# fxxJuses/MICFormer

Hardware: AMD Instinct MI355X
Metric: train volumes/sec (128^3 CT+MRI pair) (higher is better)
Workload: dtype bf16; 1 GPU; MicFormer base Head(embed_dim=48, depths 2-2-6-2, heads 3-6-12-24, window 2^3, 8 classes) full train step (fwd + MDiceLoss + bwd + Adam/cosine) on 128^3 CT+MR pairs, DropPath on; local_batch=2, global_batch=2, parallelism=dp1, launch=hipGraph replay (one graph)

## Files before the change

micformer_amd/csrc/conv3_wgradx.hip:

```cpp
#include <cstdlib>
#include <mutex>

#include "common.h"
#include "gemm_dma.h"

namespace micf {

constexpr int wCS = 48;
constexpr int wDS = 20;
constexpr int wXS = 52;
constexpr int wPairs = 27 * (wCS / 16);
constexpr int wTPW = (wPairs + 3) / 4;
constexpr int wSlabFloats = 4 * wTPW * 256;

constexpr int kWgxItems = 12;
struct WgxArgs {
  const float* dy[kWgxItems];
  const float* x1[kWgxItems]; const float* x2[kWgxItems];
  int c1, c2;
  float* ws;
  float* bias_ws;
  int B, D, H, W, tiles_d, tiles_h, tiles_w, tiles_per_group, groups, slabs, xcd_order;
};

template <int TW, bool BF16>
__global__ void __launch_bounds__(256) conv3_wgradx_kernel(WgxArgs a) {
  constexpr int CH = 16 / TW, TH = 64 / TW;
  constexpr int HH = TH + 2, HW = TW + 2, HALO = 3 * HH * HW;
  extern __shared__ __attribute__((aligned(16))) float Xs[];
  const int tid = threadIdx.x, lane = tid & 63, wave = __builtin_amdgcn_readfirstlane(tid >> 6), li = lane & 15, lr = lane >> 4;
  int slab = blockIdx.x, group = blockIdx.y;
  const int item = blockIdx.z;
  if (a.xcd_order) {
    const int L = gridDim.x * gridDim.y;
    const int lin = slab + gridDim.x * group;
    const int logical = (lin % 8) * (L / 8) + lin / 8;
    slab = logical % gridDim.x;
    group = logical / gridDim.x;
  }
  const float* __restrict__ a_dy = a.dy[item];
  const float* __restrict__ a_x1 = a.x1[item];
  const float* __restrict__ a_x2 = a.x2[item];
  const int Cin = a.c1 + a.c2;
  const int cbase = slab * wCS;
  const int64_t DHW = (int64_t)a.D * a.H * a.W;

  f32x4 acc[wTPW];
#pragma unroll
  for (int p = 0; p < wTPW; ++p) acc[p] = f32x4{0.f, 0.f, 0.f, 0.f};
  float bsum = 0.f;
  int offs[wTPW];
#pragma unroll
  for (int p = 0; p < wTPW; ++p) {
    const int pair = min(wave * wTPW + p, wPairs - 1);
    const int tap = pair / (wCS / 16), ct = pair % (wCS / 16);
    const int kd = tap / 9, kh = (tap / 3) % 3, kw = tap % 3;
    offs[p] = (((kd - 1) * HH + (kh - 1)) * HW + (kw - 1)) * wXS + ct * 16;
  }

  const int ntiles = a.B * a.tiles_d * a.tiles_h * a.tiles_w;
  const int t_begin = group * a.tiles_per_group;
  const int t_end = min(ntiles, t_begin + a.tiles_per_group);
  constexpr int NQ = HALO * (wCS / 4);
  constexpr int NB = 16;
  static_assert(NQ <= 256 * NB, "one batch per tile");
  float* Dys = Xs + HALO * wXS;
  float4 v[NB], vdy;
  auto fetch = [&](int tile) {
    int q = tile;
    const int tw = q % a.tiles_w; q /= a.tiles_w;
    const int th = q % a.tiles_h; q /= a.tiles_h;
    const int d0 = q % a.tiles_d; const int b = q / a.tiles_d;
    const int h0 = th * TH, w0 = tw * TW;
#pragma unroll
    for (int u = 0; u < NB; ++u) {
      const int idx = u * 256 + tid;
      v[u] = make_float4(0.f, 0.f, 0.f, 0.f);
      if (idx < NQ) {
        const int hv = idx / (wCS / 4), g = idx % (wCS / 4);
        const int hw = hv % HW, hh = (hv / HW) % HH, hd = hv / (HW * HH);
        const int dd = d0 + hd - 1, yy = h0 + hh - 1, ww = w0 + hw - 1;
        const int c = cbase + 4 * g;
        if ((unsigned)dd < (unsigned)a.D && (unsigned)yy < (unsigned)a.H && (unsigned)ww < (unsigned)a.W && c < Cin) {
          const int64_t tok = (int64_t)b * DHW + ((int64_t)dd * a.H + yy) * a.W + ww;
          v[u] = c < a.c1 ? *reinterpret_cast<const float4*>(a_x1 + tok * a.c1 + c)
                          : *reinterpret_cast<const float4*>(a_x2 + tok * a.c2 + (c - a.c1));
        }
      }
    }
    {
      const int tk = tid >> 2, yy = h0 + tk / TW, ww = w0 + tk % TW;
      vdy = make_float4(0.f, 0.f, 0.f, 0.f);
      if (yy < a.H && ww < a.W)
        vdy = *reinterpret_cast<const float4*>(a_dy + ((int64_t)b * DHW + ((int64_t)d0 * a.H + yy) * a.W + ww) * 16 + 4 * (tid & 3));
    }
  };
  if (t_begin < t_end) fetch(t_begin);
  for (int tile = t_begin; tile < t_end; ++tile) {
    __syncthreads();
#pragma unroll
    for (int u = 0; u < NB; ++u) {
      const int idx = u * 256 + tid;
      if (idx < NQ) *reinterpret_cast<float4*>(&Xs[(idx / (wCS / 4)) * wXS + 4 * (idx % (wCS / 4))]) = v[u];
    }
    *reinterpret_cast<float4*>(&Dys[(tid >> 2) * wDS + 4 * (tid & 3)]) = vdy;
    auto load_dy = [&](int g, float (&bv)[4]) {
#pragma unroll
      for (int s = 0; s < 4; ++s) bv[s] = g < 4 ? Dys[(g * 16 + 4 * lr + s) * wDS + li] : 0.f;
    };
    __syncthreads();
    if (tile + 1 < t_end) fetch(tile + 1);
    float bv[4], bn[4];
    load_dy(0, bv);

    if constexpr (!BF16) {
#pragma unroll 1
    for (int g = 0; g < 4; ++g) {
      load_dy(g + 1, bn);
      int vox[4];
#pragma unroll
      for (int s = 0; s < 4; ++s) {
        const int j = 4 * lr + s;
        const int lh = g * CH + j / TW, lw = j % TW;
        vox[s] = ((1 * HH + lh + 1) * HW + lw + 1) * wXS + li;
      }
      if (a.bias_ws && wave == 0) bsum += bv[0] + bv[1] + bv[2] + bv[3];
#pragma unroll
      for (int s = 0; s < 4; ++s) {
#pragma unroll
        for (int p = 0; p < wTPW; ++p) {
          acc[p] = __builtin_amdgcn_mfma_f32_16x16x4f32(Xs[vox[s] + offs[p]], bv[s], acc[p], 0, 0, 0);
        }
      }
#pragma unroll
      for (int s = 0; s < 4; ++s) bv[s] = bn[s];
    }
    } else {
#pragma unroll 1
    for (int g = 0; g < 4; g += 2) {
      float b2[4];
      load_dy(g + 1, b2);
      load_dy(g + 2, bn);
      int vox[8];
#pragma unroll
      for (int s = 0; s < 8; ++s) {
        const int j = 4 * lr + (s & 3);
        const int lh = (g + (s >> 2)) * CH + j / TW, lw = j % TW;
        vox[s] = ((1 * HH + lh + 1) * HW + lw + 1) * wXS + li;
      }
      if (a.bias_ws && wave == 0) bsum += (bv[0] + bv[1] + bv[2] + bv[3]) + (b2[0] + b2[1] + b2[2] + b2[3]);
      const bf16x8 bb = to_bf16x8(make_float4(bv[0], bv[1], bv[2], bv[3]), make_float4(b2[0], b2[1], b2[2], b2[3]));
#pragma unroll
      for (int p = 0; p < wTPW; ++p) {
        const float* xp = Xs + offs[p];
        const bf16x8 ba = to_bf16x8(make_float4(xp[vox[0]], xp[vox[1]], xp[vox[2]], xp[vox[3]]),
                                    make_float4(xp[vox[4]], xp[vox[5]], xp[vox[6]], xp[vox[7]]));
        acc[p] = __builtin_amdgcn_mfma_f32_16x16x32_bf16(ba, bb, acc[p], 0, 0, 0);
      }
#pragma unroll
      for (int s = 0; s < 4; ++s) bv[s] = bn[s];
    }
    }
  }
  float* out = a.ws + (((int64_t)item * a.slabs + slab) * a.groups + group) * wSlabFloats;
#pragma unroll
  for (int p = 0; p < wTPW; ++p)
    *reinterpret_cast<float4*>(out + ((wave * wTPW + p) * 64 + lane) * 4) = make_float4(acc[p][0], acc[p][1], acc[p][2], acc[p][3]);
  if (a.bias_ws && slab == 0 && wave == 0) {
    bsum += __shfl_xor(bsum, 16, 64);
    bsum += __shfl_xor(bsum, 32, 64);
    if (lane < 16) a.bias_ws[((int64_t)item * a.groups + group) * 16 + lane] = bsum;
  }
}

constexpr int wRSB = 104;
constexpr int wDYB = 40;
typedef short s16x4x __attribute__((ext_vector_type(4)));

__device__ __forceinline__ bf16x8 tr_pair(unsigned a0, unsigned a1) {
  const s16x4x lo = __builtin_amdgcn_ds_read_tr16_b64_v4i16((__attribute__((address_space(3))) s16x4x*)(uintptr_t)a0);
  const s16x4x hi = __builtin_amdgcn_ds_read_tr16_b64_v4i16((__attribute__((address_space(3))) s16x4x*)(uintptr_t)a1);
  return bf16x8{lo[0], lo[1], lo[2], lo[3], hi[0], hi[1], hi[2], hi[3]};
}

template <int TW>
__global__ void __launch_bounds__(256) conv3_wgradx_b16_kernel(WgxArgs a) {
  constexpr int TH = 64 / TW;
  constexpr int HH = TH + 2, HW = TW + 2, HALO = 3 * HH * HW;
  extern __shared__ __attribute__((aligned(16))) char smem[];
  const int tid = threadIdx.x, lane = tid & 63, wave = __builtin_amdgcn_readfirstlane(tid >> 6), li = lane & 15, lr = lane >> 4;
  int slab = blockIdx.x, group = blockIdx.y;
  const int item = blockIdx.z;
  if (a.xcd_order) {
    const int L = gridDim.x * gridDim.y;
    const int lin = slab + gridDim.x * group;
    const int logical = (lin % 8) * (L / 8) + lin / 8;
    slab = logical % gridDim.x;
    group = logical / gridDim.x;
  }
  const float* __restrict__ a_dy = a.dy[item];
  const float* __restrict__ a_x1 = a.x1[item];
  const float* __restrict__ a_x2 = a.x2[item];
  const int Cin = a.c1 + a.c2;
  const int cbase = slab * wCS;
  const int64_t DHW = (int64_t)a.D * a.H * a.W;
  const unsigned xh = (unsigned)(uintptr_t)smem, dyl = xh + HALO * wRSB;

  f32x4 acc[wTPW];
#pragma unroll
  for (int p = 0; p < wTPW; ++p) acc[p] = f32x4{0.f, 0.f, 0.f, 0.f};
  int offs[wTPW];
#pragma unroll
  for (int p = 0; p < wTPW; ++p) {
    const int pair = min(wave * wTPW + p, wPairs - 1);
    const int tap = pair / (wCS / 16), ct = pair % (wCS / 16);
    const int kd = tap / 9, kh = (tap / 3) % 3, kw = tap % 3;
    offs[p] = (((kd - 1) * HH + (kh - 1)) * HW + (kw - 1)) * wRSB + ct * 32;
  }
  unsigned abase[2][2], bbase[2][2];
#pragma unroll
  for (int ks = 0; ks < 2; ++ks)
#pragma unroll
    for (int r = 0; r < 2; ++r) {
      const int t = 8 * lr + 4 * r + (li >> 2);
      const int lh = ks * (32 / TW) + t / TW, lw = t % TW;
      abase[ks][r] = xh + (unsigned)(((1 * HH + lh + 1) * HW + lw + 1) * wRSB + 8 * (li & 3));
      bbase[ks][r] = dyl + (unsigned)((32 * ks + t) * wDYB + 8 * (li & 3));
    }
  float4 bs = make_float4(0.f, 0.f, 0.f, 0.f);

  const int ntiles = a.B * a.tiles_d * a.tiles_h * a.tiles_w;
  const int t_begin = group * a.tiles_per_group;
  const int t_end = min(ntiles, t_begin + a.tiles_per_group);
  constexpr int NQ = HALO * (wCS / 4);
  constexpr int NB = 16;
  static_assert(NQ <= 256 * NB, "one batch per tile");
  float4 v[NB], vdy;
  auto fetch = [&](int tile) {
    int q = tile;
    const int tw = q % a.tiles_w; q /= a.tiles_w;
    const int th = q % a.tiles_h; q /= a.tiles_h;
    const int d0 = q % a.tiles_d; const int b = q / a.tiles_d;
    const int h0 = th * TH, w0 = tw * TW;
#pragma unroll
    for (int u = 0; u < NB; ++u) {
      const int idx = u * 256 + tid;
      v[u] = make_float4(0.f, 0.f, 0.f, 0.f);
      if (idx < NQ) {
        const int hv = idx / (wCS / 4), g = idx % (wCS / 4);
        const int hw = hv % HW, hh = (hv / HW) % HH, hd = hv / (HW * HH);
        const int dd = d0 + hd - 1, yy = h0 + hh - 1, ww = w0 + hw - 1;
        const int c = cbase + 4 * g;
        if ((unsigned)dd < (unsigned)a.D && (unsigned)yy < (unsigned)a.H && (unsigned)ww < (unsigned)a.W && c < Cin) {
          const int64_t tok = (int64_t)b * DHW + ((int64_t)dd * a.H + yy) * a.W + ww;
          v[u] = c < a.c1 ? *reinterpret_cast<const float4*>(a_x1 + tok * a.c1 + c)
                          : *reinterpret_cast<const float4*>(a_x2 + tok * a.c2 + (c - a.c1));
        }
      }
    }
    const int tk = tid >> 2, yy = h0 + tk / TW, ww = w0 + tk % TW;
    vdy = make_float4(0.f, 0.f, 0.f, 0.f);
    if (yy < a.H && ww < a.W)
      vdy = *reinterpret_cast<const float4*>(a_dy + ((int64_t)b * DHW + ((int64_t)d0 * a.H + yy) * a.W + ww) * 16 + 4 * (tid & 3));
  };
  typedef unsigned u32x2w __attribute__((ext_vector_type(2)));
  if (t_begin < t_end) fetch(t_begin);
  for (int tile = t_begin; tile < t_end; ++tile) {
    __syncthreads();
#pragma unroll
    for (int u = 0; u < NB; ++u) {
      const int idx = u * 256 + tid;
      if (idx < NQ)
        *reinterpret_cast<u32x2w*>(smem + (idx / (wCS / 4)) * wRSB + 8 * (idx % (wCS / 4))) = u32x2w{pack_bf16(v[u].x, v[u].y), pack_bf16(v[u].z, v[u].w)};
    }
    *reinterpret_cast<u32x2w*>(smem + HALO * wRSB + (tid >> 2) * wDYB + 8 * (tid & 3)) = u32x2w{pack_bf16(vdy.x, vdy.y), pack_bf16(vdy.z, vdy.w)};
    bs.x += vdy.x; bs.y += vdy.y; bs.z += vdy.z; bs.w += vdy.w;
    __syncthreads();
    if (tile + 1 < t_end) fetch(tile + 1);
#pragma unroll
    for (int ks = 0; ks < 2; ++ks) {
      const bf16x8 bb = tr_pair(bbase[ks][0], bbase[ks][1]);
#pragma unroll
      for (int p = 0; p < wTPW; ++p) {
        const bf16x8 ba = tr_pair(abase[ks][0] + offs[p], abase[ks][1] + offs[p]);
        acc[p] = __builtin_amdgcn_mfma_f32_16x16x32_bf16(ba, bb, acc[p], 0, 0, 0);
      }
    }
  }
  float* out = a.ws + (((int64_t)item * a.slabs + slab) * a.groups + group) * wSlabFloats;
#pragma unroll
  for (int p = 0; p < wTPW; ++p)
    *reinterpret_cast<float4*>(out + ((wave * wTPW + p) * 64 + lane) * 4) = make_float4(acc[p][0], acc[p][1], acc[p][2], acc[p][3]);
  if (a.bias_ws && slab == 0) {
#pragma unroll
    for (int d = 4; d < 64; d <<= 1) {
      bs.x += __shfl_xor(bs.x, d, 64); bs.y += __shfl_xor(bs.y, d, 64); bs.z += __shfl_xor(bs.z, d, 64); bs.w += __shfl_xor(bs.w, d, 64);
    }
    __syncthreads();
    float* red = reinterpret_cast<float*>(smem);
    if (lane < 4) *reinterpret_cast<float4*>(red + (wave * 4 + lane) * 4) = bs;
    __syncthreads();
    if (tid < 16) a.bias_ws[((int64_t)item * a.groups + group) * 16 + tid] = red[tid] + red[16 + tid] + red[32 + tid] + red[48 + tid];
  }
}

struct WgxOut { float* dw[kWgxItems]; float* dbias[kWgxItems]; };
__global__ void __launch_bounds__(256) conv3_wgradx_reduce_kernel(const float* __restrict__ ws_all, const float* __restrict__ bias_all,
                                                                  WgxOut o, int Cin, int slabs, int groups) {
  __shared__ float red[256];
  const int item = blockIdx.y;
  const float* __restrict__ ws = ws_all + (int64_t)item * slabs * groups * wSlabFloats;
  const float* __restrict__ bias_ws = bias_all ? bias_all + (int64_t)item * groups * 16 : nullptr;
  float* __restrict__ dw = o.dw[item];
  float* __restrict__ dbias = o.dbias[item];
  const int el = threadIdx.x & 63, slice = threadIdx.x >> 6;
  const int64_t id = (int64_t)blockIdx.x * 64 + el;
  const int64_t per_slab = (int64_t)wPairs * 256;
  const bool main = id < per_slab * slabs;
  const bool bias = !main && bias_ws && dbias && id < per_slab * slabs + 16;
  float acc = 0.f;
  int slab = 0, e = 0;
  if (main) {
    slab = (int)(id / per_slab);
    e = (int)(id % per_slab);
    const float* p = ws + (int64_t)slab * groups * wSlabFloats + e;
    int g = slice;
    for (; g + 28 < groups; g += 32) {
      float v[8];
#pragma unroll
      for (int u = 0; u < 8; ++u) v[u] = p[(int64_t)(g + 4 * u) * wSlabFloats];
#pragma unroll
      for (int u = 0; u < 8; ++u) acc += v[u];
    }
    for (; g < groups; g += 4) acc += p[(int64_t)g * wSlabFloats];
  } else if (bias) {
    const int n = (int)(id - per_slab * slabs);
    for (int g = slice; g < groups; g += 4) acc += bias_ws[g * 16 + n];
  }
  red[threadIdx.x] = acc;
  __syncthreads();
  if (slice != 0) return;
  acc = red[el] + red[64 + el] + red[128 + el] + red[192 + el];
  if (main) {
    const int pair = e >> 8, lane = (e >> 2) & 63, v = e & 3;
    const int tap = pair / (wCS / 16), ct = pair % (wCS / 16);
    const int n = lane & 15, c = slab * wCS + ct * 16 + 4 * (lane >> 4) + v;
    if (c < Cin) dw[((int64_t)n * Cin + c) * 27 + tap] += acc;
  } else if (bias) {
    dbias[(int)(id - per_slab * slabs)] += acc;
  }
}

struct WgxPlan { int slabs, groups, tiles_per_group, tw; int64_t floats; };

static WgxPlan wgx_plan(int B, int D, int H, int W, int Cin, int items = 1) {
  WgxPlan p;
  p.tw = W >= 12 ? 16 : 8;
  const int th = 64 / p.tw;
  const int ntiles = B * D * ((H + th - 1) / th) * ((W + p.tw - 1) / p.tw);
  p.slabs = (Cin + wCS - 1) / wCS;
  constexpr int wg_target = 256;
  int groups = (wg_target + p.slabs * items - 1) / (p.slabs * items);
  if (groups < 4) groups = 4 < ntiles ? 4 : ntiles;
  if (groups > ntiles) groups = ntiles;
  p.tiles_per_group = (ntiles + groups - 1) / groups;
  p.groups = (ntiles + p.tiles_per_group - 1) / p.tiles_per_group;
  p.floats = (int64_t)p.slabs * p.groups * wSlabFloats + (int64_t)p.groups * 16;
  return p;
}

int64_t conv3_wgradx_workspace(int B, int D, int H, int W, int N, int c1, int c2, int items) {
  if (N != 16 || W < 4 || (c1 & 3) || (c2 & 3) || items < 1 || items > kWgxItems) return 0;
  return wgx_plan(B, D, H, W, c1 + c2, items).floats * items;
}

int conv3_wgradx_items(const float* const* dy, const float* const* x1, const float* const* x2, float* const* dw, float* const* dbias,
                       int n, int c1, int c2, int B, int D, int H, int W, int N, float* ws, int64_t ws_floats, hipStream_t stream,
                       int dtype) {
  const int64_t need = conv3_wgradx_workspace(B, D, H, W, N, c1, c2, n);
  if (need == 0 || !ws || ws_floats < need || !aligned16(ws)) return MICF_EUNSUPPORTED;
  const WgxPlan p = wgx_plan(B, D, H, W, c1 + c2, n);
  WgxArgs a{};
  WgxOut o{};
  bool any_bias = false;
  for (int i = 0; i < n; ++i) {
    if (!dy[i] || !x1[i] || !dw[i] || !aligned16(dy[i]) || !aligned16(x1[i]) || (x2 && x2[i] && !aligned16(x2[i]))) return MICF_EUNSUPPORTED;
    a.dy[i] = dy[i]; a.x1[i] = x1[i]; a.x2[i] = (x2 && x2[i]) ? x2[i] : x1[i];
    o.dw[i] = dw[i]; o.dbias[i] = dbias ? dbias[i] : nullptr;
    any_bias = any_bias || o.dbias[i];
  }
  a.c1 = c1; a.c2 = c2;
  a.ws = ws; a.bias_ws = any_bias ? ws + (int64_t)n * p.slabs * p.groups * wSlabFloats : nullptr;
  a.B = B; a.D = D; a.H = H; a.W = W;
  const int th = 64 / p.tw;
  a.tiles_d = D; a.tiles_h = (H + th - 1) / th; a.tiles_w = (W + p.tw - 1) / p.tw;
  a.tiles_per_group = p.tiles_per_group; a.groups = p.groups; a.slabs = p.slabs;
  a.xcd_order = ((p.slabs * p.groups) % 8 == 0) ? 1 : 0;
  static std::once_flag attr_once;
  std::call_once(attr_once, [] {
    (void)hipFuncSetAttribute(reinterpret_cast<const void*>(&conv3_wgradx_kernel<16, false>), hipFuncAttributeMaxDynamicSharedMemorySize, 80 * 1024);
    (void)hipFuncSetAttribute(reinterpret_cast<const void*>(&conv3_wgradx_kernel<8, false>), hipFuncAttributeMaxDynamicSharedMemorySize, 80 * 1024);
    (void)hipFuncSetAttribute(reinterpret_cast<const void*>(&conv3_wgradx_b16_kernel<16>), hipFuncAttributeMaxDynamicSharedMemorySize, 64 * 1024);
    (void)hipFuncSetAttribute(reinterpret_cast<const void*>(&conv3_wgradx_b16_kernel<8>), hipFuncAttributeMaxDynamicSharedMemorySize, 64 * 1024);
  });
  const dim3 grid(p.slabs, p.groups, n);
  if (p.tw == 16) {
    constexpr int HALO = 3 * (4 + 2) * (16 + 2);
    if (dtype == MICF_DTYPE_BF16) hipLaunchKernelGGL((conv3_wgradx_b16_kernel<16>), grid, dim3(256), HALO * wRSB + 64 * wDYB, stream, a);
    else hipLaunchKernelGGL((conv3_wgradx_kernel<16, false>), grid, dim3(256), sizeof(float) * (HALO * wXS + 64 * wDS), stream, a);
  } else {
    constexpr int HALO = 3 * (8 + 2) * (8 + 2);
    if (dtype == MICF_DTYPE_BF16) hipLaunchKernelGGL((conv3_wgradx_b16_kernel<8>), grid, dim3(256), HALO * wRSB + 64 * wDYB, stream, a);
    else hipLaunchKernelGGL((conv3_wgradx_kernel<8, false>), grid, dim3(256), sizeof(float) * (HALO * wXS + 64 * wDS), stream, a);
  }
  if (hipGetLastError() != hipSuccess) return MICF_ELAUNCH;
  const int64_t ne = (int64_t)wPairs * 256 * p.slabs + 16;
  hipLaunchKernelGGL(conv3_wgradx_reduce_kernel, dim3((unsigned)((ne + 63) / 64), n), dim3(256), 0, stream, ws, a.bias_ws, o,
                     c1 + c2, p.slabs, p.groups);
  return hipGetLastError() == hipSuccess ? MICF_OK : MICF_ELAUNCH;
}

int conv3_wgradx(const float* dy, const float* x1, int c1, const float* x2, int c2, float* dw, float* dbias, int B, int D, int H,
                 int W, int N, float* ws, int64_t ws_floats, hipStream_t stream, int dtype) {
  return conv3_wgradx_items(&dy, &x1, &x2, &dw, &dbias, 1, c1, c2, B, D, H, W, N, ws, ws_floats, stream, dtype);
}

}
```

Baseline: 230.8 pairs/s.

## Use 8-wave blocks in bf16 conv3 wgrad and write final-layout partials

The bf16 3x3x3 weight-gradient kernel now runs 512-thread blocks, so each wave holds fewer tap/channel accumulator tiles and the halo prefetch needs fewer registers per thread. At the end, each block transposes its accumulators through LDS into the final [N][Cin][27] weight layout. A simpler per-element sum kernel then adds the group partials, replacing the slab-aware reduce kernel. The group count now rounds down instead of up, and only half the threads load dy, which trades some load balance for less register pressure and a cheaper reduction.

```diff
diff --git a/micformer_amd/csrc/conv3_wgradx.hip b/micformer_amd/csrc/conv3_wgradx.hip
--- a/micformer_amd/csrc/conv3_wgradx.hip
+++ b/micformer_amd/csrc/conv3_wgradx.hip
@@ -175,6 +175,8 @@
 
 constexpr int wRSB = 104;
 constexpr int wDYB = 40;
+constexpr int wBWaves = 8;
+constexpr int wBTPW = (wPairs + wBWaves - 1) / wBWaves;
 typedef short s16x4x __attribute__((ext_vector_type(4)));
 
 __device__ __forceinline__ bf16x8 tr_pair(unsigned a0, unsigned a1) {
@@ -184,9 +186,11 @@
 }
 
 template <int TW>
-__global__ void __launch_bounds__(256) conv3_wgradx_b16_kernel(WgxArgs a) {
+__global__ void __launch_bounds__(64 * wBWaves) conv3_wgradx_b16_kernel(WgxArgs a) {
+  constexpr int NT = 64 * wBWaves;
   constexpr int TH = 64 / TW;
   constexpr int HH = TH + 2, HW = TW + 2, HALO = 3 * HH * HW;
+  static_assert(16 * 16 * 27 * 4 <= HALO * wRSB + 64 * wDYB, "one channel tile of the slab fits the staging LDS");
   extern __shared__ __attribute__((aligned(16))) char smem[];
   const int tid = threadIdx.x, lane = tid & 63, wave = __builtin_amdgcn_readfirstlane(tid >> 6), li = lane & 15, lr = lane >> 4;
   int slab = blockIdx.x, group = blockIdx.y;
@@ -206,13 +210,13 @@
   const int64_t DHW = (int64_t)a.D * a.H * a.W;
   const unsigned xh = (unsigned)(uintptr_t)smem, dyl = xh + HALO * wRSB;
 
-  f32x4 acc[wTPW];
-#pragma unroll
-  for (int p = 0; p < wTPW; ++p) acc[p] = f32x4{0.f, 0.f, 0.f, 0.f};
-  int offs[wTPW];
-#pragma unroll
-  for (int p = 0; p < wTPW; ++p) {
-    const int pair = min(wave * wTPW + p, wPairs - 1);
+  f32x4 acc[wBTPW];
+#pragma unroll
+  for (int p = 0; p < wBTPW; ++p) acc[p] = f32x4{0.f, 0.f, 0.f, 0.f};
+  int offs[wBTPW];
+#pragma unroll
+  for (int p = 0; p < wBTPW; ++p) {
+    const int pair = min(wave * wBTPW + p, wPairs - 1);
     const int tap = pair / (wCS / 16), ct = pair % (wCS / 16);
     const int kd = tap / 9, kh = (tap / 3) % 3, kw = tap % 3;
     offs[p] = (((kd - 1) * HH + (kh - 1)) * HW + (kw - 1)) * wRSB + ct * 32;
@@ -233,8 +237,9 @@
   const int t_begin = group * a.tiles_per_group;
   const int t_end = min(ntiles, t_begin + a.tiles_per_group);
   constexpr int NQ = HALO * (wCS / 4);
-  constexpr int NB = 16;
-  static_assert(NQ <= 256 * NB, "one batch per tile");
+  constexpr int NB = (NQ + NT - 1) / NT;
+  static_assert(NB <= 8, "halo prefetch registers");
+  const bool dy_thread = tid < 256;
   float4 v[NB], vdy;
   auto fetch = [&](int tile) {
     int q = tile;
@@ -244,7 +249,7 @@
     const int h0 = th * TH, w0 = tw * TW;
 #pragma unroll
     for (int u = 0; u < NB; ++u) {
-      const int idx = u * 256 + tid;
+      const int idx = u * NT + tid;
       v[u] = make_float4(0.f, 0.f, 0.f, 0.f);
       if (idx < NQ) {
         const int hv = idx / (wCS / 4), g = idx % (wCS / 4);
@@ -258,9 +263,9 @@
         }
       }
     }
-    const int tk = tid >> 2, yy = h0 + tk / TW, ww = w0 + tk % TW;
+    const int tk = (tid & 255) >> 2, yy = h0 + tk / TW, ww = w0 + tk % TW;
     vdy = make_float4(0.f, 0.f, 0.f, 0.f);
-    if (yy < a.H && ww < a.W)
+    if (dy_thread && yy < a.H && ww < a.W)
       vdy = *reinterpret_cast<const float4*>(a_dy + ((int64_t)b * DHW + ((int64_t)d0 * a.H + yy) * a.W + ww) * 16 + 4 * (tid & 3));
   };
   typedef unsigned u32x2w __attribute__((ext_vector_type(2)));
@@ -269,11 +274,12 @@
     __syncthreads();
 #pragma unroll
     for (int u = 0; u < NB; ++u) {
-      const int idx = u * 256 + tid;
+      const int idx = u * NT + tid;
       if (idx < NQ)
         *reinterpret_cast<u32x2w*>(smem + (idx / (wCS / 4)) * wRSB + 8 * (idx % (wCS / 4))) = u32x2w{pack_bf16(v[u].x, v[u].y), pack_bf16(v[u].z, v[u].w)};
     }
-    *reinterpret_cast<u32x2w*>(smem + HALO * wRSB + (tid >> 2) * wDYB + 8 * (tid & 3)) = u32x2w{pack_bf16(vdy.x, vdy.y), pack_bf16(vdy.z, vdy.w)};
+    if (dy_thread)
+      *reinterpret_cast<u32x2w*>(smem + HALO * wRSB + (tid >> 2) * wDYB + 8 * (tid & 3)) = u32x2w{pack_bf16(vdy.x, vdy.y), pack_bf16(vdy.z, vdy.w)};
     bs.x += vdy.x; bs.y += vdy.y; bs.z += vdy.z; bs.w += vdy.w;
     __syncthreads();
     if (tile + 1 < t_end) fetch(tile + 1);
@@ -281,30 +287,71 @@
     for (int ks = 0; ks < 2; ++ks) {
       const bf16x8 bb = tr_pair(bbase[ks][0], bbase[ks][1]);
 #pragma unroll
-      for (int p = 0; p < wTPW; ++p) {
+      for (int p = 0; p < wBTPW; ++p) {
         const bf16x8 ba = tr_pair(abase[ks][0] + offs[p], abase[ks][1] + offs[p]);
         acc[p] = __builtin_amdgcn_mfma_f32_16x16x32_bf16(ba, bb, acc[p], 0, 0, 0);
       }
     }
   }
-  float* out = a.ws + (((int64_t)item * a.slabs + slab) * a.groups + group) * wSlabFloats;
-#pragma unroll
-  for (int p = 0; p < wTPW; ++p)
-    *reinterpret_cast<float4*>(out + ((wave * wTPW + p) * 64 + lane) * 4) = make_float4(acc[p][0], acc[p][1], acc[p][2], acc[p][3]);
+  float* __restrict__ out = a.ws + ((int64_t)item * a.groups + group) * 16 * Cin * 27;
+  float* red = reinterpret_cast<float*>(smem);
+#pragma unroll 1
+  for (int ct = 0; ct < wCS / 16; ++ct) {
+    __syncthreads();
+#pragma unroll
+    for (int p = 0; p < wBTPW; ++p) {
+      const int pair = wave * wBTPW + p;
+      if (pair < wPairs && pair % (wCS / 16) == ct) {
+        const int tap = pair / (wCS / 16);
+#pragma unroll
+        for (int e = 0; e < 4; ++e) red[(li * 16 + 4 * lr + e) * 27 + tap] = acc[p][e];
+      }
+    }
+    __syncthreads();
+    const int c0 = cbase + ct * 16;
+    for (int i = tid; i < 16 * 16 * 27; i += NT) {
+      const int n = i / (16 * 27), r = i % (16 * 27);
+      if (c0 + r / 27 < Cin) out[((int64_t)n * Cin + c0) * 27 + r] = red[i];
+    }
+  }
   if (a.bias_ws && slab == 0) {
 #pragma unroll
     for (int d = 4; d < 64; d <<= 1) {
       bs.x += __shfl_xor(bs.x, d, 64); bs.y += __shfl_xor(bs.y, d, 64); bs.z += __shfl_xor(bs.z, d, 64); bs.w += __shfl_xor(bs.w, d, 64);
     }
     __syncthreads();
-    float* red = reinterpret_cast<float*>(smem);
-    if (lane < 4) *reinterpret_cast<float4*>(red + (wave * 4 + lane) * 4) = bs;
+    if (lane < 4 && wave < 4) *reinterpret_cast<float4*>(red + (wave * 4 + lane) * 4) = bs;
     __syncthreads();
     if (tid < 16) a.bias_ws[((int64_t)item * a.groups + group) * 16 + tid] = red[tid] + red[16 + tid] + red[32 + tid] + red[48 + tid];
   }
 }
 
 struct WgxOut { float* dw[kWgxItems]; float* dbias[kWgxItems]; };
+__global__ void __launch_bounds__(256) conv3_wgradx_b16_sum_kernel(const float* __restrict__ ws_all, const float* __restrict__ bias_all,
+                                                                   WgxOut o, int len, int groups) {
+  const int item = blockIdx.y;
+  const int i = blockIdx.x * 256 + threadIdx.x;
+  if (i < len) {
+    const float* __restrict__ p = ws_all + (int64_t)item * groups * len + i;
+    float s = 0.f;
+    int g = 0;
+    for (; g + 8 <= groups; g += 8) {
+      float v[8];
+#pragma unroll
+      for (int u = 0; u < 8; ++u) v[u] = p[(int64_t)(g + u) * len];
+#pragma unroll
+      for (int u = 0; u < 8; ++u) s += v[u];
+    }
+    for (; g < groups; ++g) s += p[(int64_t)g * len];
+    o.dw[item][i] += s;
+  } else if (i < len + 16 && bias_all && o.dbias[item]) {
+    const float* __restrict__ bw = bias_all + (int64_t)item * groups * 16 + (i - len);
+    float s = 0.f;
+    for (int g = 0; g < groups; ++g) s += bw[g * 16];
+    o.dbias[item][i - len] += s;
+  }
+}
+
 __global__ void __launch_bounds__(256) conv3_wgradx_reduce_kernel(const float* __restrict__ ws_all, const float* __restrict__ bias_all,
                                                                   WgxOut o, int Cin, int slabs, int groups) {
   __shared__ float red[256];
@@ -360,7 +407,7 @@
   const int ntiles = B * D * ((H + th - 1) / th) * ((W + p.tw - 1) / p.tw);
   p.slabs = (Cin + wCS - 1) / wCS;
   constexpr int wg_target = 256;
-  int groups = (wg_target + p.slabs * items - 1) / (p.slabs * items);
+  int groups = wg_target / (p.slabs * items);
   if (groups < 4) groups = 4 < ntiles ? 4 : ntiles;
   if (groups > ntiles) groups = ntiles;
   p.tiles_per_group = (ntiles + groups - 1) / groups;
@@ -406,14 +453,20 @@
   const dim3 grid(p.slabs, p.groups, n);
   if (p.tw == 16) {
     constexpr int HALO = 3 * (4 + 2) * (16 + 2);
-    if (dtype == MICF_DTYPE_BF16) hipLaunchKernelGGL((conv3_wgradx_b16_kernel<16>), grid, dim3(256), HALO * wRSB + 64 * wDYB, stream, a);
+    if (dtype == MICF_DTYPE_BF16) hipLaunchKernelGGL((conv3_wgradx_b16_kernel<16>), grid, dim3(64 * wBWaves), HALO * wRSB + 64 * wDYB, stream, a);
     else hipLaunchKernelGGL((conv3_wgradx_kernel<16, false>), grid, dim3(256), sizeof(float) * (HALO * wXS + 64 * wDS), stream, a);
   } else {
     constexpr int HALO = 3 * (8 + 2) * (8 + 2);
-    if (dtype == MICF_DTYPE_BF16) hipLaunchKernelGGL((conv3_wgradx_b16_kernel<8>), grid, dim3(256), HALO * wRSB + 64 * wDYB, stream, a);
+    if (dtype == MICF_DTYPE_BF16) hipLaunchKernelGGL((conv3_wgradx_b16_kernel<8>), grid, dim3(64 * wBWaves), HALO * wRSB + 64 * wDYB, stream, a);
     else hipLaunchKernelGGL((conv3_wgradx_kernel<8, false>), grid, dim3(256), sizeof(float) * (HALO * wXS + 64 * wDS), stream, a);
   }
   if (hipGetLastError() != hipSuccess) return MICF_ELAUNCH;
+  if (dtype == MICF_DTYPE_BF16) {
+    const int len = 16 * (c1 + c2) * 27;
+    hipLaunchKernelGGL(conv3_wgradx_b16_sum_kernel, dim3((unsigned)((len + 16 + 255) / 256), n), dim3(256), 0, stream, ws, a.bias_ws, o,
+                       len, p.groups);
+    return hipGetLastError() == hipSuccess ? MICF_OK : MICF_ELAUNCH;
+  }
   const int64_t ne = (int64_t)wPairs * 256 * p.slabs + 16;
   hipLaunchKernelGGL(conv3_wgradx_reduce_kernel, dim3((unsigned)((ne + 63) / 64), n), dim3(256), 0, stream, ws, a.bias_ws, o,
                      c1 + c2, p.slabs, p.groups);
```

Measured after the change: 232.9 pairs/s (median of 6 runs). Within noise of the previous version (+0.9%).
